# PinataFarms/FEARTracker

Hardware: AMD Instinct MI355X
Metric: search-region crops/sec (FEAR-XS 256x256) (higher is better)
Workload: dtype f32; 1 GPU; FEAR-XS track(): batch=256 synthetic 256x256 search / 128x128 template crops per GPU, fp32; batch_per_gpu=256, global_batch=256, weights=FEAR-XS-NoEmbs (fp16 values upcast to fp32), engine_pass=256, parallelism=dp1, math=fp32 MFMA (v_mfma_f32_16x16x4_f32), exact fp32

## Files before the change

### feartracker_amd/csrc/fear_e1pair.h

```cpp
#pragma once
#include <type_traits>
#include <vector>

#ifndef E1P_NA
#define E1P_NA 3
#endif

namespace fear {

struct E1PairArgs {
    const float* X;
    float* Y;
    const float* Wpk;
    int H, W, tiles_x, tiles_y;
    int tpw;
};

struct E1PairGeom {
    static constexpr int C = 24, T = 16, XW = T + 4, MW = T + 2, NQ = C / 4;
    static constexpr int XPL = XW * XW * 4;
    static constexpr int XSKEW = 12;
    static constexpr int xb(int q) { return q * XPL + (q >> 1) * XSKEW; }
    static constexpr int XT_FLOATS = NQ * XPL + 2 * XSKEW;
    static constexpr int NSLOT = NQ * XW * XW, NIT = (NSLOT + 511) / 512;
    static constexpr int MPL = (MW * MW * 4 + 63) / 64 * 64;
    static constexpr int NPIX_A = MW * MW, NMT_A = (NPIX_A + 15) / 16, MTA = (NMT_A + 7) / 8;
    static constexpr int FRAG = 4 * 256, TAP0 = FRAG, TAP1 = TAP0 + 9 * 16, BD = TAP1 + 9 * 8, BP = BD + 24, WBLK = BP + 32;
    static constexpr int WS = WBLK - FRAG;
    static_assert(WS % 4 == 0 && WBLK % 4 == 0, "16-byte granules");
    static constexpr int LDS_FLOATS = XT_FLOATS + NQ * MPL + 2 * WS;
    static constexpr int LDS_BYTES = LDS_FLOATS * 4;
};

inline void e1pair_pack_block(std::vector<float>& out, const float* dw, const float* bd, const float* pw, const float* bp) {
    using G = E1PairGeom;
    for (int c = 0; c < 2; ++c)
        for (int nt = 0; nt < 2; ++nt)
            for (int l = 0; l < 64; ++l)
                for (int i = 0; i < 4; ++i) {
                    const int n = nt * 16 + (l & 15);
                    const int k = c == 0 ? (l >> 4) * 4 + i : (i < 2 ? 16 + 2 * (l >> 4) + i : G::C);
                    out.push_back(n < G::C && k < G::C ? pw[n * G::C + k] : 0.f);
                }
    for (int t = 0; t < 9; ++t)
        for (int ch = 0; ch < 16; ++ch) out.push_back(dw[ch * 9 + t]);
    for (int t = 0; t < 9; ++t)
        for (int ch = 16; ch < 24; ++ch) out.push_back(dw[ch * 9 + t]);
    for (int ch = 0; ch < 24; ++ch) out.push_back(bd ? bd[ch] : 0.f);
    for (int ch = 0; ch < 32; ++ch) out.push_back(ch < 24 ? bp[ch] : 0.f);
}

__device__ __forceinline__ void pk_fma2(f32x2& d, const f32x2& a, const f32x2& b) {
    asm volatile("v_pk_fma_f32 %0, %1, %2, %0" : "+v"(d) : "v"(a), "v"(b));
}

__device__ __forceinline__ void e1_project(f32x4 d4, f32x2 d2, const f32x4 (&wp)[4], const f32x4 (&bias)[2], f32x4 (&acc)[2]) {
    d4.x = fmaxf(d4.x, 0.f); d4.y = fmaxf(d4.y, 0.f); d4.z = fmaxf(d4.z, 0.f); d4.w = fmaxf(d4.w, 0.f);
    d2.x = fmaxf(d2.x, 0.f); d2.y = fmaxf(d2.y, 0.f);
#pragma unroll
    for (int nt = 0; nt < 2; ++nt) {
        f32x4 a = bias[nt];
#pragma unroll
        for (int q = 0; q < 4; ++q) a = __builtin_amdgcn_mfma_f32_16x16x4f32(wp[nt][q], d4[q], a, 0, 0, 0);
#pragma unroll
        for (int q = 0; q < 2; ++q) a = __builtin_amdgcn_mfma_f32_16x16x4f32(wp[2 + nt][q], d2[q], a, 0, 0, 0);
        acc[nt] = a;
    }
}

__device__ __forceinline__ int e1_fill_slot(int tid) {
    const int l = tid & 63, g = l >> 3, j = l & 7;
    return (tid & ~63) | (8 * ((g + j) & 7) + j);
}

template <int IT0, int IT1>
__device__ __forceinline__ void e1_issue_loads(const E1PairArgs& a, unsigned tix, int tid, f32x4 (&xv)[E1PairGeom::NIT]) {
    using G = E1PairGeom;
    constexpr int T = G::T, XW = G::XW, NQ = G::NQ, C = G::C;
    const int tiles = a.tiles_x * a.tiles_y;
    const long crop = tix / tiles;
    const int tile = tix % tiles;
    const int ox0 = (tile % a.tiles_x) * T, oy0 = (tile / a.tiles_x) * T;
    const float* Xc = a.X + crop * a.H * a.W * C;
    const __amdgpu_buffer_rsrc_t img = __builtin_amdgcn_make_buffer_rsrc(const_cast<float*>(Xc), 0, a.H * a.W * C * 4, 0x00020000);
    int t = e1_fill_slot(tid);
    asm volatile("" : "+v"(t));
#pragma unroll
    for (int it = IT0; it < IT1; ++it) {
        const int s = it * 512 + t;
        const int pix = s / NQ, q = s - pix * NQ;
        const int py = pix / XW, px = pix - py * XW;
        const int gy = oy0 - 2 + py, gx = ox0 - 2 + px;
        const bool ok = s < G::NSLOT && gy >= 0 && gy < a.H && gx >= 0 && gx < a.W;
        xv[it] = __builtin_bit_cast(f32x4, __builtin_amdgcn_raw_buffer_load_b128(img, ok ? ((gy * a.W + gx) * C + q * 4) * 4 : (int)0x80000000, 0, 0));
    }
}
template <int IT0, int IT1>
__device__ __forceinline__ void e1_commit_tile(float* Xt, int tid, const f32x4 (&xv)[E1PairGeom::NIT]) {
    using G = E1PairGeom;
    int t = e1_fill_slot(tid);
    asm volatile("" : "+v"(t));
#pragma unroll
    for (int it = IT0; it < IT1; ++it) {
        const int s = it * 512 + t;
        const int pix = s / G::NQ, q = s - pix * G::NQ;
        if (s < G::NSLOT) *reinterpret_cast<f32x4*>(Xt + q * G::XPL + (q >> 1) * G::XSKEW + pix * 4) = xv[it];
    }
}

__global__ __launch_bounds__(512, 4) void e1pair_kernel(E1PairArgs a) {
    using G = E1PairGeom;
    constexpr int T = G::T, XW = G::XW, MW = G::MW, XPL = G::XPL, MPL = G::MPL, NQ = G::NQ, C = G::C;
    extern __shared__ __attribute__((aligned(16))) float lds[];
    float* const Xt = lds;
    float* const Mt = lds + G::XT_FLOATS;
    float* const WSl = Mt + NQ * MPL;
    const int tid = threadIdx.x, lane = tid & 63;
    const int wave = __builtin_amdgcn_readfirstlane(tid >> 6);
    const int li = lane & 15, lk = lane >> 4;
    const int tiles = a.tiles_x * a.tiles_y;
    const int tpw = a.tpw > 0 ? a.tpw : 1;
    const unsigned t_first = xcd_tile_index(blockIdx.x, gridDim.x) * (unsigned)tpw;

    constexpr int NIT = G::NIT;
    constexpr int NA = E1P_NA;
    f32x4 xv0[NIT];
    e1_issue_loads<0, NIT>(a, t_first, tid, xv0);
    auto load_wp = [&](int b, f32x4 (&wp)[4]) {
#pragma unroll
        for (int f = 0; f < 4; ++f) wp[f] = *reinterpret_cast<const f32x4*>(a.Wpk + b * G::WBLK + f * 256 + lane * 4);
    };
    if (tid < 2 * G::WS / 4) {
        const int b = tid / (G::WS / 4), j = tid - b * (G::WS / 4);
        *reinterpret_cast<f32x4*>(WSl + b * G::WS + j * 4) = *reinterpret_cast<const f32x4*>(a.Wpk + b * G::WBLK + G::FRAG + j * 4);
    }
    e1_commit_tile<0, NIT>(Xt, tid, xv0);

    for (int ti = 0; ti < tpw; ++ti) {
        const unsigned tix = t_first + ti;
        const long crop = tix / tiles;
        const int tile = tix % tiles;
        const int ox0 = (tile % a.tiles_x) * T, oy0 = (tile / a.tiles_x) * T;
        float* Yc = a.Y + crop * a.H * a.W * C;
        __syncthreads();
        f32x4 xv[NIT];
        int li_o = li, lk_o = lk;
        asm volatile("" : "+v"(li_o), "+v"(lk_o));
        if (ti + 1 < tpw) e1_issue_loads<0, NA>(a, tix + 1, tid, xv);

        {
            const float* ws = WSl;
            f32x4 wp[4];
            load_wp(0, wp);
            auto block_a = [&](auto nm_tag) {
                constexpr int NM = decltype(nm_tag)::value;
                int pc[NM], cpix[NM];
                bool valid[NM];
                float inside[NM];
#pragma unroll
                for (int i = 0; i < NM; ++i) {
                    const int mt = wave + 8 * i;
                    const int j = (mt - MW) * 16 + li_o;
                    valid[i] = mt < MW || j < 2 * MW;
                    const int my = mt < MW ? mt : (valid[i] ? j >> 1 : 0), mx = mt < MW ? li_o : 16 + (j & 1);
                    pc[i] = my * MW + mx;
                    cpix[i] = (my + 1) * XW + mx + 1;
                    const int gy = oy0 - 1 + my, gx = ox0 - 1 + mx;
                    inside[i] = (gy >= 0 && gy < a.H && gx >= 0 && gx < a.W) ? 1.f : 0.f;
                }
                f32x4 d4[NM];
                f32x2 d2[NM];
                {
                    const f32x4 b0 = *reinterpret_cast<const f32x4*>(ws + (G::BD - G::FRAG) + lk_o * 4);
                    const f32x2 b1 = *reinterpret_cast<const f32x2*>(ws + (G::BD - G::FRAG) + 16 + lk_o * 2);
#pragma unroll
                    for (int i = 0; i < NM; ++i) { d4[i] = b0; d2[i] = b1; }
                }
                const float* s0 = Xt + lk_o * XPL + (lk_o >> 1) * G::XSKEW;
                const float* s1 = Xt + (4 + (lk_o >> 1)) * XPL + 2 * G::XSKEW + (lk_o & 1) * 2;
#pragma unroll
                for (int k = 0; k < 9; ++k) {
                    const f32x4 w4 = *reinterpret_cast<const f32x4*>(ws + (G::TAP0 - G::FRAG) + k * 16 + lk_o * 4);
                    const f32x2 w2 = *reinterpret_cast<const f32x2*>(ws + (G::TAP1 - G::FRAG) + k * 8 + lk_o * 2);
                    const int off = ((k / 3 - 1) * XW + (k % 3 - 1)) * 4;
#pragma unroll
                    for (int i = 0; i < NM; ++i) {
                        const f32x4 v4 = *reinterpret_cast<const f32x4*>(s0 + cpix[i] * 4 + off);
                        const f32x2 v2 = *reinterpret_cast<const f32x2*>(s1 + cpix[i] * 4 + off);
                        pk_fma4(d4[i], v4, w4);
                        pk_fma2(d2[i], v2, w2);
                    }
                }
                f32x4 bpv[2];
#pragma unroll
                for (int nt = 0; nt < 2; ++nt) bpv[nt] = *reinterpret_cast<const f32x4*>(ws + (G::BP - G::FRAG) + (nt * 4 + lk_o) * 4);
#pragma unroll
                for (int i = 0; i < NM; ++i) {
                    f32x4 acc[2];
                    e1_project(d4[i], d2[i], wp, bpv, acc);
#pragma unroll
                    for (int nt = 0; nt < 2; ++nt) {
                        if (nt == 1 && lk_o >= 2) continue;
                        const int qd = nt * 4 + lk_o;
                        const f32x4 v = (acc[nt] + *reinterpret_cast<const f32x4*>(Xt + qd * XPL + (qd >> 1) * G::XSKEW + cpix[i] * 4)) * inside[i];
                        if (valid[i]) *reinterpret_cast<f32x4*>(Mt + qd * MPL + pc[i] * 4) = v;
                    }
                }
            };
            if (wave + 16 < G::NMT_A) block_a(std::integral_constant<int, 3>{});
            else block_a(std::integral_constant<int, 2>{});
        }
        __syncthreads();
        if (ti + 1 < tpw) { e1_commit_tile<0, NA>(Xt, tid, xv); e1_issue_loads<NA, NIT>(a, tix + 1, tid, xv); }

        {
            const float* ws = WSl + G::WS;
            f32x4 wp[4];
            load_wp(1, wp);
            f32x4 bpv[2];
#pragma unroll
            for (int nt = 0; nt < 2; ++nt) bpv[nt] = *reinterpret_cast<const f32x4*>(ws + (G::BP - G::FRAG) + (nt * 4 + lk_o) * 4);
            const int row0 = wave * 2;
            const int cpix = (row0 + 1) * MW + li_o + 1;
            f32x4 d4[2];
            f32x2 d2[2];
            d4[0] = d4[1] = *reinterpret_cast<const f32x4*>(ws + (G::BD - G::FRAG) + lk_o * 4);
            d2[0] = d2[1] = *reinterpret_cast<const f32x2*>(ws + (G::BD - G::FRAG) + 16 + lk_o * 2);
            {
                const float* s0 = Mt + lk_o * MPL + cpix * 4;
                const float* s1 = Mt + (4 + (lk_o >> 1)) * MPL + cpix * 4 + (lk_o & 1) * 2;
                f32x4 w4[2][3];
                f32x2 w2[2][3];
#pragma unroll
                for (int iy = 0; iy < 4; ++iy) {
#pragma unroll
                    for (int kx = 0; kx < 3; ++kx) {
                        if (iy < 3) {
                            w4[iy & 1][kx] = *reinterpret_cast<const f32x4*>(ws + (G::TAP0 - G::FRAG) + (iy * 3 + kx) * 16 + lk_o * 4);
                            w2[iy & 1][kx] = *reinterpret_cast<const f32x2*>(ws + (G::TAP1 - G::FRAG) + (iy * 3 + kx) * 8 + lk_o * 2);
                        }
                        const int off = ((iy - 1) * MW + (kx - 1)) * 4;
                        const f32x4 v4 = *reinterpret_cast<const f32x4*>(s0 + off);
                        const f32x2 v2 = *reinterpret_cast<const f32x2*>(s1 + off);
                        if (iy < 3) { pk_fma4(d4[0], v4, w4[iy & 1][kx]); pk_fma2(d2[0], v2, w2[iy & 1][kx]); }
                        if (iy >= 1) { pk_fma4(d4[1], v4, w4[(iy - 1) & 1][kx]); pk_fma2(d2[1], v2, w2[(iy - 1) & 1][kx]); }
                    }
                }
            }
            const unsigned ylane = (unsigned)(li_o * C + lk_o * 4);
#pragma unroll
            for (int r = 0; r < 2; ++r) {
                f32x4 acc[2];
                e1_project(d4[r], d2[r], wp, bpv, acc);
                float* yrow = Yc + ((long)(oy0 + row0 + r) * a.W + ox0) * C;
#pragma unroll
                for (int nt = 0; nt < 2; ++nt) {
                    if (nt == 1 && lk_o >= 2) continue;
                    const int qd = nt * 4 + lk_o;
                    const f32x4 v = acc[nt] + *reinterpret_cast<const f32x4*>(Mt + qd * MPL + (cpix + r * MW) * 4);
                    *reinterpret_cast<f32x4*>(yrow + (ylane + (unsigned)(nt * 16))) = v;
                }
            }
        }
        if (ti + 1 < tpw) e1_commit_tile<NA, NIT>(Xt, tid, xv);
    }
}

}
```

### feartracker_amd/csrc/fear_engine.hip

```cpp
#include <hip/hip_runtime.h>

#include <atomic>
#include <cstdio>
#include <cstdlib>
#include <cstring>
#include <map>
#include <memory>
#include <mutex>
#include <string>
#include <vector>

#include "../../include/fear_hip.h"
#include "../../include/fearw_format.h"
#include "fear_kernels.h"
#include "fear_headchain.h"
#include "fear_headchain_b.h"
#include "fear_e1pair.h"
#include "fear_chain32.h"
#include "fear_yuv.h"
#ifndef FEAR_E1PAIR_TPW_MAX
#define FEAR_E1PAIR_TPW_MAX 1
#endif

namespace {

using namespace fear;

float half_to_float(uint16_t h) {
    const uint32_t sign = (uint32_t)(h & 0x8000u) << 16;
    uint32_t exp = (h >> 10) & 0x1f;
    uint32_t man = h & 0x3ffu;
    uint32_t bits;
    if (exp == 0) {
        if (man == 0) {
            bits = sign;
        } else {
            int e = -1;
            do { ++e; man <<= 1; } while (!(man & 0x400u));
            bits = sign | ((uint32_t)(127 - 15 - e) << 23) | ((man & 0x3ffu) << 13);
        }
    } else if (exp == 31) {
        bits = sign | 0x7f800000u | (man << 13);
    } else {
        bits = sign | ((exp + 127 - 15) << 23) | (man << 13);
    }
    float f;
    memcpy(&f, &bits, 4);
    return f;
}

uint16_t float_to_half(float f) {
    uint32_t x;
    memcpy(&x, &f, 4);
    const uint32_t sign = (x >> 16) & 0x8000u;
    const int32_t e = (int32_t)((x >> 23) & 0xff) - 127 + 15;
    uint32_t man = x & 0x7fffffu;
    if (((x >> 23) & 0xff) == 0xff) return (uint16_t)(sign | 0x7c00u | (man ? 0x200u : 0));
    if (e >= 31) return (uint16_t)(sign | 0x7c00u);
    if (e <= 0) {
        if (e < -10) return (uint16_t)sign;
        man |= 0x800000u;
        const int shift = 14 - e;
        uint32_t h = man >> shift;
        const uint32_t rem = man & ((1u << shift) - 1), half = 1u << (shift - 1);
        if (rem > half || (rem == half && (h & 1))) ++h;
        return (uint16_t)(sign | h);
    }
    uint32_t h = ((uint32_t)e << 10) | (man >> 13);
    const uint32_t rem = man & 0x1fffu;
    if (rem > 0x1000u || (rem == 0x1000u && (h & 1))) ++h;
    return (uint16_t)(sign | h);
}

uint16_t float_to_bf16(float f) {
    uint32_t x;
    memcpy(&x, &f, 4);
    if ((x & 0x7f800000u) == 0x7f800000u) return (uint16_t)((x >> 16) | ((x & 0xffffu) ? 0x40u : 0));
    x += 0x7fffu + ((x >> 16) & 1u);
    return (uint16_t)(x >> 16);
}

struct Conv {
    int cout, cin_g, groups, k, stride, pad, relu, has_bias;
    std::vector<float> w;
    std::vector<float> b;
    float* d_w = nullptr;
    float* d_w2 = nullptr;
    float* d_b = nullptr;
    bool is_dw() const { return groups == cout && cin_g == 1 && groups > 1; }
    bool is_pw() const { return groups == 1 && k == 1; }
};

struct Fused16Row;
struct TileRow;
struct TileK;

enum OpType { OP_STEM, OP_PW, OP_DW, OP_CORR, OP_PW_SMALL, OP_IR16, OP_IRTILE, OP_CHAIN16, OP_HEADCHAIN, OP_E1PAIR, OP_CHAIN32, OP_CHAIN32_16 };

struct Op {
    OpType type;
    int conv = -1;
    int in_buf = -1, in_ld = 0, in_off = 0;
    int out_buf = -1, out_ld = 0, out_off = 0;
    int res_buf = -1, res_ld = 0;
    int H = 0, W = 0;
    int Ho = 0, Wo = 0;
    int C = 0, N = 0;
    int relu = 0, act = 0;
    int out_external = 0;
    int tmpl_cls = 0;
    int pred_fused = 0;
    float* pred_packed = nullptr;
    int pred_conv_p = -1;
    int pw_split = 0;
    int splitk = 0;
    int tiny = 0;
    int nsplit = 0;
    int part_buf = -1;
    int lane = 0;
    int corr_fused = 0;
    int conv_e = -1, conv_d = -1, conv_p = -1;
    int relu_dw = 0;
    const Fused16Row* f16 = nullptr;
    const TileRow* tile = nullptr;
    const TileK* tk = nullptr;
    float* d_packed = nullptr;
    int math = 0;
    int pred_cout = 0;
    int stem = 0;
    int io_bf16 = 0;
    float* chain_pk[8] = {nullptr};
    int chain_cp[8] = {0};
    float* chain16_pk[8] = {nullptr};
    int chain16_cp[8] = {0};
    float* neck_pk = nullptr;
    int neck_conv = -1;
    float* hc_w[2][4] = {{nullptr}};
    float* hc_wd0[2] = {nullptr};
    float* hc_wdc[2] = {nullptr};
    float* hc_pred[2] = {nullptr};
    float* hc_taps[2][4] = {{nullptr}};
    int hc_pred_conv[2] = {-1, -1};
    int hc_pred_act[2] = {0, 0};
    char name[64];
    double flops = 0, bytes = 0;
    std::vector<std::pair<hipEvent_t, hipEvent_t>> events;
    double prof_ms = 0;
    int64_t prof_n = 0;
};

enum class PlanKind {
    Throughput,
    Small,
    Tiny,
    MidSize,
};

struct Plan {
    bool with_head = false;
    bool small = false;
    std::vector<Op> ops;
    int head_first = -1;
    int n_bufs = 0;
    size_t buf_floats_per_crop = 0;
};

}

struct fear_handle {
    int device = 0;
    std::vector<Conv> convs;
    std::vector<FearwBlock> blocks;
    bool has_head = false;
    int feat_channels = 0;
    int max_batch = 64;
// ... 1222 lines not shown
                if (!h->event_pool.empty()) { *e = h->event_pool.back(); h->event_pool.pop_back(); }
                else HIP_TRY(h, hipEventCreate(e));
            }
            HIP_TRY(h, hipEventRecord(e0, s));
        }
        const Conv* c = op.conv >= 0 ? &h->convs[op.conv] : nullptr;
        switch (op.type) {
            case OP_STEM: {
                if (h->fuse && op.Wo % 16 == 0) {
                    StemMfmaArgs a{ext.img, c->d_w2, c->d_b, buf(op.out_buf), n, op.H, op.W, op.Ho, op.Wo};
                    const long rows = (long)n * op.Ho;
                    hipLaunchKernelGGL(stem_mfma_kernel, dim3((rows + 3) / 4), dim3(256), 0, s, a);
                } else {
                    StemArgs a{ext.img, c->d_w, c->d_b, buf(op.out_buf), n, op.H, op.W, op.Ho, op.Wo};
                    const long total = (long)n * op.Ho * op.Wo;
                    hipLaunchKernelGGL(stem_conv_kernel, dim3((total + 255) / 256), dim3(256), 0, s, a);
                }
                break;
            }
            case OP_PW: {
                PwArgs a{};
                a.X = buf(op.in_buf) + op.in_off; a.ldx = op.in_ld;
                a.W = c->d_w; a.bias = c->d_b;
                a.R = op.res_buf >= 0 ? buf(op.res_buf) : nullptr; a.ldr = op.res_ld;
                a.M = n * op.H * op.W; a.K = op.C; a.N = op.N; a.relu = op.relu;
                if (op.out_external == 1) { a.Y = ext.feat_out; a.ldy = op.N; a.nchw_hw = op.H * op.W; }
                else { a.Y = buf(op.out_buf) + op.out_off; a.ldy = op.out_ld; a.nchw_hw = 0; }
                const int n_tiles = (op.N + 15) / 16;
                int nt = pick_nt(n_tiles);
                const int rows_per_block = 4 * 2 * 16;
                dim3 grid((a.M + rows_per_block - 1) / rows_per_block);
                if (op.pw_split && n_tiles % 2 == 0) {
                    grid.y = n_tiles / 2;
                    hipLaunchKernelGGL((pw_mfma_kernel<2, 2, false, 8>), grid, dim3(256), 0, s, a);
                    break;
                }
                if (h->math && p.with_head) launch_pw_h<false>(h->math, n_tiles, grid, s, a);
                else launch_pw_nt<2, false>(nt, grid, s, a);
                break;
            }
            case OP_CORR: {
                PwArgs a{};
                a.X = buf(op.in_buf) + op.in_off; a.ldx = op.in_ld;
                a.W = (op.tmpl_cls && ext.tmpl_cls) ? ext.tmpl_cls : ext.tmpl;
                a.bias = nullptr; a.R = nullptr;
                a.Y = buf(op.out_buf) + op.out_off; a.ldy = op.out_ld;
                a.M = n * op.H * op.W; a.K = op.C; a.N = op.N; a.relu = 0; a.nchw_hw = 0;
                a.rows_per_crop = op.H * op.W; a.w_crop_stride = (long)op.C * op.N;
                const int rows_per_block = 4 * 2 * 16;
                dim3 grid((a.M + rows_per_block - 1) / rows_per_block);
                int nt = pick_nt(op.N / 16);
                if (op.pw_split) {
                    grid.x = (a.M + 63) / 64;
                    grid.y = op.N / 16;
                    if (a.K <= 256) hipLaunchKernelGGL((pw_mfma_kernel<1, 1, true, 16>), grid, dim3(256), 0, s, a);
                    else hipLaunchKernelGGL((pw_mfma_kernel<1, 1, true, 8>), grid, dim3(256), 0, s, a);
                    break;
                }
                if (h->math) launch_pw_h<true>(h->math, op.N / 16, grid, s, a);
                else launch_pw_nt<2, true>(nt, grid, s, a);
                break;
            }
            case OP_DW: {
                DwArgs a{};
                a.X = buf(op.in_buf) + op.in_off; a.ldx = op.in_ld;
                a.Wt = c->d_w; a.bias = c->d_b;
                a.Y = buf(op.out_buf); a.ldy = op.out_ld;
                a.B = n; a.H = op.H; a.W = op.W; a.C = op.C; a.Ho = op.Ho; a.Wo = op.Wo; a.relu = op.relu;
                const long strips = (op.Ho + 3) / 4;
                const long total = (long)n * strips * op.Wo * (op.C / 4);
                dim3 grid((total + 255) / 256);
                launch_dw(c->k, c->stride, grid, s, a);
                break;
            }
            case OP_IR16: {
                const Fused16Row& r = *op.f16;
                const F16K& f = r.by_math(op.math);
                Ir2Args a{};
                a.X = buf(op.in_buf) + op.in_off; a.ldx = op.in_ld;
                a.Wpk = op.d_packed; a.bp = h->convs[op.conv_p].d_b;
                a.R = op.res_buf >= 0 ? buf(op.res_buf) : nullptr; a.ldr = op.res_ld;
                a.Y = op.out_buf >= 0 ? buf(op.out_buf) : nullptr; a.ldy = op.out_ld;
                a.relu_dw = op.relu_dw; a.relu_out = op.relu;
                if (op.pred_cout > 0) {
                    a.pred_cout = op.pred_cout; a.pred_act = op.act;
                    a.pred_stride = op.out_external == 3 ? ext.cls_stride : ext.bbox_stride;
                    float* y = op.out_external == 3 ? ext.cls_out : ext.bbox_out;
                    if (op.pred_fused) { a.P_Wpk = op.pred_packed; a.P_bp = h->convs[op.pred_conv_p].d_b; a.P_Y = y; }
                    else a.Y = y;
                }
                if (op.nsplit) {
                    const Conv& dconv = h->convs[op.conv_d];
                    a.nsplit_wstride = (long)(dconv.cout / 16) * (256 + dconv.k * dconv.k * 16 + 16);
                    if (op.tiny) hipLaunchKernelGGL(r.tiny.kernel, dim3(n, op.nsplit, 16 / kTinyRows), dim3(64 * kTinyRows * kTinyKSplit), r.tiny.lds_bytes, s, a);
                    else hipLaunchKernelGGL(f.kernel, dim3(n, op.nsplit), dim3(512), f.lds_bytes, s, a);
                } else if (op.tiny) {
                    hipLaunchKernelGGL(r.tiny.kernel, dim3(n, 1, 16 / kTinyRows), dim3(64 * kTinyRows * kTinyKSplit), r.tiny.lds_bytes, s, a);
                } else if (op.splitk) {
                    Ir2Args pa = a;
                    const Conv& dconv = h->convs[op.conv_d];
                    pa.kc_count = dconv.cout / 16 / op.splitk;
                    pa.Y = buf(op.part_buf); pa.ldy = op.N;
                    pa.kc_part_stride = (long)n * 256 * op.N;
                    pa.R = nullptr;
                    hipLaunchKernelGGL(r.splitk.kernel, dim3(n, op.splitk), dim3(512), r.splitk.lds_bytes, s, pa);
                    SplitKReduceArgs ra{};
                    ra.P = pa.Y; ra.bias = a.bp; ra.R = a.R; ra.Y = a.Y; ra.part_stride = pa.kc_part_stride;
                    ra.W = op.splitk; ra.M = n * 256; ra.N = op.N; ra.ldp = op.N; ra.ldr = a.ldr; ra.ldy = a.ldy; ra.relu = a.relu_out;
                    const long total = (long)ra.M * (ra.N / 4);
                    hipLaunchKernelGGL(splitk_reduce_kernel, dim3((unsigned)((total + 255) / 256)), dim3(256), 0, s, ra);
                } else if (op.corr_fused) {
                    a.Z = (op.tmpl_cls && ext.tmpl_cls) ? ext.tmpl_cls : ext.tmpl;
                    a.z_stride = (long)kCorrC * kCorrTz;
                    hipLaunchKernelGGL(kSep16CorrKernel, dim3(n), dim3(512), kSep16CorrLds, s, a);
                } else if (op.pred_fused) {
                    hipLaunchKernelGGL(kSep16PredKernel, dim3(n), dim3(512), kSep16PredLds, s, a);
                } else {
                    hipLaunchKernelGGL(f.kernel, dim3(n), dim3(512), f.lds_bytes, s, a);
                }
                break;
            }
            case OP_IRTILE: {
                const TileK& f = *op.tk;
                IrT2Args ta{};
                Ir2Args& a = ta.b;
                if (op.stem) { a.X = ext.img; a.ldx = 0; }
                else { a.X = buf(op.in_buf) + op.in_off; a.ldx = op.in_ld; }
                a.Wpk = op.d_packed; a.bp = h->convs[op.conv_p].d_b;
                a.R = op.res_buf >= 0 ? buf(op.res_buf) : nullptr; a.ldr = op.res_ld;
                a.Y = buf(op.out_buf); a.ldy = op.out_ld;
                a.relu_dw = op.relu_dw; a.relu_out = op.relu;
                ta.H = op.H; ta.W = op.W; ta.tiles_x = op.Wo / f.tw; ta.tiles_y = op.Ho / f.th;
                if (op.splitk) {
                    const TileK& ks = op.tile->ksplit;
                    SplitKReduceArgs ra{};
                    ra.bias = a.bp; ra.R = a.R; ra.Y = a.Y; ra.W = op.splitk; ra.M = n * op.Ho * op.Wo; ra.N = op.N; ra.ldp = op.N;
                    ra.ldr = a.ldr; ra.ldy = a.ldy; ra.relu = a.relu_out;
                    ra.part_stride = (long)ra.M * op.N;
                    a.Y = buf(op.part_buf); a.ldy = op.N; a.R = nullptr; a.kc_part_stride = ra.part_stride;
                    ra.P = a.Y;
                    hipLaunchKernelGGL(ks.kernel, dim3((unsigned)n * ta.tiles_x * ta.tiles_y, op.splitk), dim3(512), ks.lds_bytes, s, ta);
                    const long total = (long)ra.M * (ra.N / 4);
                    hipLaunchKernelGGL(splitk_reduce_kernel, dim3((unsigned)((total + 255) / 256)), dim3(256), 0, s, ra);
                    break;
                }
                const TileK& k = op.io_bf16 ? *op.tile->io_variant(op.io_bf16) : f;
                hipLaunchKernelGGL(k.kernel, dim3((unsigned)n * ta.tiles_x * ta.tiles_y), dim3(64 * k.nw), k.lds_bytes, s, ta);
                break;
            }
            case OP_E1PAIR: {
                E1PairArgs a{};
                a.X = buf(op.in_buf); a.Y = buf(op.out_buf); a.Wpk = op.d_packed;
                a.H = op.H; a.W = op.W; a.tiles_x = op.W / E1PairGeom::T; a.tiles_y = op.H / E1PairGeom::T;
                const unsigned total = (unsigned)n * a.tiles_x * a.tiles_y;
                a.tpw = 1;
                for (int t = FEAR_E1PAIR_TPW_MAX; t > 1; t >>= 1)
                    if (total % t == 0 && total / t >= 512) { a.tpw = t; break; }
                hipLaunchKernelGGL(e1pair_kernel, dim3(total / a.tpw), dim3(512), E1PairGeom::LDS_BYTES, s, a);
                break;
            }
            case OP_CHAIN16: {
                Chain16Args a{};
                a.X = buf(op.in_buf) + op.in_off; a.ldx = op.in_ld;
                a.Y = buf(op.out_buf); a.ldy = op.out_ld;
                for (int j = 0; j < 7; ++j) { a.Wpk[j] = op.chain_pk[j]; a.bp[j] = h->convs[op.chain_cp[j]].d_b; }
                a.neck_pk = op.neck_pk; a.neck_b = h->convs[op.neck_conv].d_b;
                hipLaunchKernelGGL(kChainXSKernel, dim3(n), dim3(512), kChainXSLds, s, a);
                break;
            }
            case OP_CHAIN32: {
                Chain32Args a{};
                a.X = buf(op.in_buf) + op.in_off; a.ldx = op.in_ld;
                a.Y = buf(op.out_buf); a.ldy = op.out_ld;
                for (int j = 0; j < 4; ++j) { a.Wpk[j] = op.chain_pk[j]; a.bp[j] = h->convs[op.chain_cp[j]].d_b; }
                hipLaunchKernelGGL(kChain32XSKernel, dim3(n), dim3(512), C32Geom::LDS_BYTES, s, a);
                break;
            }
            case OP_CHAIN32_16: {
                Chain32Args a{};
                a.X = buf(op.in_buf) + op.in_off; a.ldx = op.in_ld;
                a.Y = nullptr; a.ldy = 0;
                for (int j = 0; j < 4; ++j) { a.Wpk[j] = op.chain_pk[j]; a.bp[j] = h->convs[op.chain_cp[j]].d_b; }
                Chain16Args b{};
                b.X = nullptr; b.ldx = 0;
                b.Y = buf(op.out_buf); b.ldy = op.out_ld;
                for (int j = 0; j < 7; ++j) { b.Wpk[j] = op.chain16_pk[j]; b.bp[j] = h->convs[op.chain16_cp[j]].d_b; }
                b.neck_pk = op.neck_pk; b.neck_b = h->convs[op.neck_conv].d_b;
                hipLaunchKernelGGL(kChain32_16XSKernel, dim3(n), dim3(512), kChain32_16Lds, s, a, b);
                break;
            }
            case OP_HEADCHAIN: {
                if (op.math == 2) {
                    HeadChainBArgs a{};
                    a.X = buf(op.in_buf) + op.in_off; a.ldx = op.in_ld; a.n_crops = n;
                    a.relu_dw = op.relu_dw; a.relu_out = op.relu;
                    for (int br = 0; br < 2; ++br) {
                        HeadChainBBranch& b = a.br[br];
                        for (int l = 0; l < 4; ++l) { b.W[l] = op.hc_w[br][l]; b.Wd[l] = op.hc_taps[br][l]; }
                        b.Z = (br == 0 && ext.tmpl_cls) ? ext.tmpl_cls : ext.tmpl;
                        b.z_stride = (long)HeadChainG::C * HeadChainG::TZ;
                        b.P_W = op.hc_pred[br]; b.P_bp = h->convs[op.hc_pred_conv[br]].d_b;
                        b.P_Y = br == 0 ? ext.cls_out : ext.bbox_out;
                        b.pred_stride = br == 0 ? ext.cls_stride : ext.bbox_stride;
                        b.pred_cout = br == 0 ? 1 : 4; b.pred_act = op.hc_pred_act[br];
                    }
                    hipLaunchKernelGGL(kHeadChainBKernel, dim3(16u * ((unsigned)(n + 7) / 8)), dim3(512), HeadChainBG::LDS_BYTES, s, a);
                    break;
                }
                HeadChainArgs a{};
                a.X = buf(op.in_buf) + op.in_off; a.ldx = op.in_ld; a.n_crops = n;
                a.relu_dw = op.relu_dw; a.relu_out = op.relu;
                for (int br = 0; br < 2; ++br) {
                    HeadChainBranch& b = a.br[br];
                    for (int l = 0; l < 4; ++l) b.W[l] = op.hc_w[br][l];
                    b.Wd0 = op.hc_wd0[br]; b.WdC = op.hc_wdc[br];
                    b.Z = (br == 0 && ext.tmpl_cls) ? ext.tmpl_cls : ext.tmpl;
                    b.z_stride = (long)HeadChainG::C * HeadChainG::TZ;
                    b.P_Wpk = op.hc_pred[br]; b.P_bp = h->convs[op.hc_pred_conv[br]].d_b;
                    b.P_Y = br == 0 ? ext.cls_out : ext.bbox_out;
                    b.pred_stride = br == 0 ? ext.cls_stride : ext.bbox_stride;
                    b.pred_cout = br == 0 ? 1 : 4; b.pred_act = op.hc_pred_act[br];
                    b.D = buf(op.out_buf) + (size_t)br * n * HeadChainG::D_FLOATS;
                }
                hipLaunchKernelGGL(kHeadChainKernel, dim3(16u * ((unsigned)(n + 7) / 8)), dim3(512), HeadChainG::LDS_BYTES, s, a);
                break;
            }
            case OP_PW_SMALL: {
                PwSmallArgs a{};
                a.X = buf(op.in_buf); a.ldx = op.in_ld; a.W = c->d_w; a.bias = c->d_b;
                a.Y = op.out_external == 3 ? ext.cls_out : ext.bbox_out;
                a.M = n * op.H * op.W; a.K = op.C; a.N = op.N; a.hw = op.H * op.W; a.act = op.act;
                a.crop_stride = op.out_external == 3 ? ext.cls_stride : ext.bbox_stride;
                dim3 grid(((long)a.M * 16 + 255) / 256);
                if (op.N == 1) hipLaunchKernelGGL((pw_small_kernel<1>), grid, dim3(256), 0, s, a);
                else hipLaunchKernelGGL((pw_small_kernel<4>), grid, dim3(256), 0, s, a);
                break;
            }
        }
        if (prof) {
            HIP_TRY(h, hipEventRecord(e1, s));
            op.events.emplace_back(e0, e1);
        }
    }
    if (forked) {
        HIP_TRY(h, hipEventRecord(h->branch_join, h->branch_stream));
        HIP_TRY(h, hipStreamWaitEvent(s_main, h->branch_join, 0));
    }
    HIP_TRY(h, hipGetLastError());
    return FEAR_OK;
}

int drain_events(fear_handle* h) {
    for (auto& kv : h->plans)
        for (Op& op : kv.second->ops) {
            for (auto& ev : op.events) {
                HIP_TRY(h, hipEventSynchronize(ev.second));
                float ms = 0.f;
                HIP_TRY(h, hipEventElapsedTime(&ms, ev.first, ev.second));
                op.prof_ms += ms;
                op.prof_n += 1;
                h->event_pool.push_back(ev.first);
                h->event_pool.push_back(ev.second);
            }
            op.events.clear();
        }
    return FEAR_OK;
}

int drop_plans(fear_handle* h) {
    if (h->plans.empty() && h->plan_allocs.empty()) return FEAR_OK;
    HIP_TRY(h, hipSetDevice(h->device));
    HIP_TRY(h, hipDeviceSynchronize());
    const int st = drain_events(h);
    if (st != FEAR_OK) return st;
    h->plans.clear();
    for (float* p : h->plan_allocs) hipFree(p);
    h->plan_allocs.clear();
    return FEAR_OK;
}

struct OptionDesc {
    int option;
    int fear_handle::*field;
    int64_t min, max;
    bool rebuilds_plans;
};
const OptionDesc kOptions[] = {
    {FEAR_OPT_MAX_BATCH, &fear_handle::max_batch, 1, 65536, false},
    {FEAR_OPT_PROFILE, &fear_handle::profile, 0, 1, false},
    {FEAR_OPT_PROFILE_OP, &fear_handle::profile_op, -1, 4096, false},
    {FEAR_OPT_FUSE, &fear_handle::fuse, 0, 1, true},
    {FEAR_OPT_MATH, &fear_handle::math, 0, 2, true},
    {FEAR_OPT_CHAIN, &fear_handle::chain, 0, 1, true},
    {FEAR_OPT_SMALL_PASS, &fear_handle::small_pass, 0, 65536, false},
    {FEAR_OPT_PLAN_CROPS, &fear_handle::plan_crops, 0, 65536, false},
    {FEAR_OPT_DUAL_HEAD, &fear_handle::dual_head, 0, 1, true},
    {FEAR_OPT_TILE_V4, &fear_handle::tile_v4, 0, 1, true},
    {FEAR_OPT_TINY_SEP, &fear_handle::tiny_sep, 0, 1, true},
    {FEAR_OPT_HEAD_STAGGER, &fear_handle::head_stagger_us, 0, 1000, false},
    {FEAR_OPT_HEAD_CHAIN, &fear_handle::head_chain, 0, 1, true},
    {FEAR_OPT_E1_PAIR, &fear_handle::e1_pair, 0, 1, true},
    {FEAR_OPT_CHAIN32, &fear_handle::chain32, 0, 2, true},
    {FEAR_OPT_BF16_STORE, &fear_handle::bf16_store, 0, 1, true},
    {FEAR_OPT_SPLIT_STREAMS, &fear_handle::split_streams, 0, 1, false},
};
const OptionDesc* find_option(int option) {
    for (const OptionDesc& d : kOptions)
        if (d.option == option) return &d;
    return nullptr;
}

// ... 401 lines not shown
```

Baseline: 118,400 crops/s.

## Simplify e1pair to one tile per block with row-based buffer fills

Drops the multi-tile-per-block software pipeline, which was inactive by default since TPW_MAX was 1, so each block now handles a single tile. The halo fill is reorganised so two waves load one input row, using per-row buffer resources with a scalar row offset and a lane-skewed slot order, replacing per-slot divides and bounds checks. Stage A precomputes LDS pointers per output row and splits row and column sub-tiles, and the per-lane weight offsets are hoisted into registers. The aim is less address arithmetic and fewer VGPRs in the fill and stencil loops, and the fill now depends on RSLOT fitting within 128 slots.

Measured after the change: 118,900 crops/s (median of 6 runs). Within noise of the previous version (+0.4%).

```diff
diff --git a/feartracker_amd/csrc/fear_e1pair.h b/feartracker_amd/csrc/fear_e1pair.h
--- a/feartracker_amd/csrc/fear_e1pair.h
+++ b/feartracker_amd/csrc/fear_e1pair.h
@@ -2,8 +2,10 @@
 #include <type_traits>
 #include <vector>
 
-#ifndef E1P_NA
-#define E1P_NA 3
+#if defined(__HIPCC__)
+#define E1P_HD __host__ __device__
+#else
+#define E1P_HD
 #endif
 
 namespace fear {
@@ -13,16 +15,17 @@
     float* Y;
     const float* Wpk;
     int H, W, tiles_x, tiles_y;
-    int tpw;
 };
 
 struct E1PairGeom {
     static constexpr int C = 24, T = 16, XW = T + 4, MW = T + 2, NQ = C / 4;
     static constexpr int XPL = XW * XW * 4;
     static constexpr int XSKEW = 12;
-    static constexpr int xb(int q) { return q * XPL + (q >> 1) * XSKEW; }
+    static constexpr E1P_HD int xb(int q) { return q * XPL + (q >> 1) * XSKEW; }
     static constexpr int XT_FLOATS = NQ * XPL + 2 * XSKEW;
-    static constexpr int NSLOT = NQ * XW * XW, NIT = (NSLOT + 511) / 512;
+    static constexpr int RSLOT = NQ * XW;
+    static constexpr int NSLOT = RSLOT * XW, NIT = XW / 4;
+    static_assert(XW % 4 == 0 && RSLOT <= 128, "eight waves fill four rows per pass, two waves a row");
     static constexpr int MPL = (MW * MW * 4 + 63) / 64 * 64;
     static constexpr int NPIX_A = MW * MW, NMT_A = (NPIX_A + 15) / 16, MTA = (NMT_A + 7) / 8;
     static constexpr int FRAG = 4 * 256, TAP0 = FRAG, TAP1 = TAP0 + 9 * 16, BD = TAP1 + 9 * 8, BP = BD + 24, WBLK = BP + 32;
@@ -31,6 +34,36 @@
     static constexpr int LDS_FLOATS = XT_FLOATS + NQ * MPL + 2 * WS;
     static constexpr int LDS_BYTES = LDS_FLOATS * 4;
 };
+
+constexpr E1P_HD int e1_fill_slot_of_lane(int lane) { return (lane * 9) & 63; }
+constexpr E1P_HD int e1_fill_row_slot(int tid) { return ((tid >> 6) & 1) * 64 + e1_fill_slot_of_lane(tid & 63); }
+constexpr E1P_HD int e1_fill_pix(int tid) { return e1_fill_row_slot(tid) / E1PairGeom::NQ; }
+constexpr E1P_HD int e1_fill_quad(int tid) { return e1_fill_row_slot(tid) % E1PairGeom::NQ; }
+constexpr E1P_HD int e1_fill_row(int tid, int it) { return it * 4 + (tid >> 7); }
+constexpr E1P_HD int e1_fill_lds_thread(int tid) {
+    return E1PairGeom::xb(e1_fill_quad(tid)) + ((tid >> 7) * E1PairGeom::XW + e1_fill_pix(tid)) * 4;
+}
+constexpr E1P_HD int e1_fill_lds_pass(int it) { return it * 4 * E1PairGeom::XW * 4; }
+constexpr E1P_HD int e1_fill_base_bytes(int ox0) { return (ox0 - 2) * E1PairGeom::C * 4; }
+constexpr E1P_HD int e1_fill_row_bytes(int gy, int W) { return gy * W * E1PairGeom::C * 4; }
+constexpr E1P_HD int e1_fill_lane_bytes(int tid) { return e1_fill_row_slot(tid) * 16; }
+constexpr E1P_HD bool e1_fill_lane_ok(int tid, int ox0, int W) {
+    const int gx = ox0 - 2 + e1_fill_pix(tid);
+    return e1_fill_row_slot(tid) < E1PairGeom::RSLOT && gx >= 0 && gx < W;
+}
+constexpr E1P_HD bool e1_fill_row_ok(int tid, int it, int oy0, int H) {
+    const int gy = oy0 - 2 + e1_fill_row(tid, it);
+    return gy >= 0 && gy < H;
+}
+
+constexpr E1P_HD int e1_a_row_xpix(int wave, int li) { return (wave + 1) * E1PairGeom::XW + li + 1; }
+constexpr E1P_HD int e1_a_row_mpix(int wave, int li) { return wave * E1PairGeom::MW + li; }
+struct E1ColLane { bool valid; int my, mx; };
+constexpr E1P_HD E1ColLane e1_a_col_lane(int c, int li) {
+    const int j = c * 16 + li;
+    const bool valid = j < 2 * E1PairGeom::MW;
+    return {valid, valid ? j >> 1 : 0, 16 + (j & 1)};
+}
 
 inline void e1pair_pack_block(std::vector<float>& out, const float* dw, const float* bd, const float* pw, const float* bp) {
     using G = E1PairGeom;
@@ -50,6 +83,8 @@
     for (int ch = 0; ch < 32; ++ch) out.push_back(ch < 24 ? bp[ch] : 0.f);
 }
 
+#if defined(__HIPCC__)
+
 __device__ __forceinline__ void pk_fma2(f32x2& d, const f32x2& a, const f32x2& b) {
     asm volatile("v_pk_fma_f32 %0, %1, %2, %0" : "+v"(d) : "v"(a), "v"(b));
 }
@@ -68,49 +103,9 @@
     }
 }
 
-__device__ __forceinline__ int e1_fill_slot(int tid) {
-    const int l = tid & 63, g = l >> 3, j = l & 7;
-    return (tid & ~63) | (8 * ((g + j) & 7) + j);
-}
-
-template <int IT0, int IT1>
-__device__ __forceinline__ void e1_issue_loads(const E1PairArgs& a, unsigned tix, int tid, f32x4 (&xv)[E1PairGeom::NIT]) {
-    using G = E1PairGeom;
-    constexpr int T = G::T, XW = G::XW, NQ = G::NQ, C = G::C;
-    const int tiles = a.tiles_x * a.tiles_y;
-    const long crop = tix / tiles;
-    const int tile = tix % tiles;
-    const int ox0 = (tile % a.tiles_x) * T, oy0 = (tile / a.tiles_x) * T;
-    const float* Xc = a.X + crop * a.H * a.W * C;
-    const __amdgpu_buffer_rsrc_t img = __builtin_amdgcn_make_buffer_rsrc(const_cast<float*>(Xc), 0, a.H * a.W * C * 4, 0x00020000);
-    int t = e1_fill_slot(tid);
-    asm volatile("" : "+v"(t));
-#pragma unroll
-    for (int it = IT0; it < IT1; ++it) {
-        const int s = it * 512 + t;
-        const int pix = s / NQ, q = s - pix * NQ;
-        const int py = pix / XW, px = pix - py * XW;
-        const int gy = oy0 - 2 + py, gx = ox0 - 2 + px;
-        const bool ok = s < G::NSLOT && gy >= 0 && gy < a.H && gx >= 0 && gx < a.W;
-        xv[it] = __builtin_bit_cast(f32x4, __builtin_amdgcn_raw_buffer_load_b128(img, ok ? ((gy * a.W + gx) * C + q * 4) * 4 : (int)0x80000000, 0, 0));
-    }
-}
-template <int IT0, int IT1>
-__device__ __forceinline__ void e1_commit_tile(float* Xt, int tid, const f32x4 (&xv)[E1PairGeom::NIT]) {
-    using G = E1PairGeom;
-    int t = e1_fill_slot(tid);
-    asm volatile("" : "+v"(t));
-#pragma unroll
-    for (int it = IT0; it < IT1; ++it) {
-        const int s = it * 512 + t;
-        const int pix = s / G::NQ, q = s - pix * G::NQ;
-        if (s < G::NSLOT) *reinterpret_cast<f32x4*>(Xt + q * G::XPL + (q >> 1) * G::XSKEW + pix * 4) = xv[it];
-    }
-}
-
 __global__ __launch_bounds__(512, 4) void e1pair_kernel(E1PairArgs a) {
     using G = E1PairGeom;
-    constexpr int T = G::T, XW = G::XW, MW = G::MW, XPL = G::XPL, MPL = G::MPL, NQ = G::NQ, C = G::C;
+    constexpr int T = G::T, XW = G::XW, MW = G::MW, XPL = G::XPL, MPL = G::MPL, NQ = G::NQ, C = G::C, NIT = G::NIT;
     extern __shared__ __attribute__((aligned(16))) float lds[];
     float* const Xt = lds;
     float* const Mt = lds + G::XT_FLOATS;
@@ -119,151 +114,181 @@
     const int wave = __builtin_amdgcn_readfirstlane(tid >> 6);
     const int li = lane & 15, lk = lane >> 4;
     const int tiles = a.tiles_x * a.tiles_y;
-    const int tpw = a.tpw > 0 ? a.tpw : 1;
-    const unsigned t_first = xcd_tile_index(blockIdx.x, gridDim.x) * (unsigned)tpw;
-
-    constexpr int NIT = G::NIT;
-    constexpr int NA = E1P_NA;
-    f32x4 xv0[NIT];
-    e1_issue_loads<0, NIT>(a, t_first, tid, xv0);
+    const unsigned tix = xcd_tile_index(blockIdx.x, gridDim.x);
+    const long crop = tix / tiles;
+    const int tile = tix % tiles;
+    const int ox0 = (tile % a.tiles_x) * T, oy0 = (tile / a.tiles_x) * T;
+    const float* Xc = a.X + crop * a.H * a.W * C;
+    float* Yc = a.Y + crop * a.H * a.W * C;
+
+    {
+        const int ftid = wave * 64 + lane;
+        const int voff = e1_fill_lane_ok(ftid, ox0, a.W) ? e1_fill_lane_bytes(ftid) : (int)0x80000000;
+        const char* xrow0 = reinterpret_cast<const char*>(Xc) + e1_fill_base_bytes(ox0);
+        f32x4 xv[NIT];
+#pragma unroll
+        for (int it = 0; it < NIT; ++it) {
+            const bool rok = e1_fill_row_ok(wave * 64, it, oy0, a.H);
+            const int gy = oy0 - 2 + e1_fill_row(wave * 64, it);
+            const int soff = rok ? e1_fill_row_bytes(gy, a.W) : 0;
+            const __amdgpu_buffer_rsrc_t img = __builtin_amdgcn_make_buffer_rsrc(const_cast<char*>(xrow0), 0, rok ? soff + G::RSLOT * 16 : 0, 0x00020000);
+            xv[it] = __builtin_bit_cast(f32x4, __builtin_amdgcn_raw_buffer_load_b128(img, voff, soff, 0));
+        }
+        if (tid < 2 * G::WS / 4) {
+            const int b = tid >= G::WS / 4 ? 1 : 0, j = tid - b * (G::WS / 4);
+            *reinterpret_cast<f32x4*>(WSl + b * G::WS + j * 4) = *reinterpret_cast<const f32x4*>(a.Wpk + b * G::WBLK + G::FRAG + j * 4);
+        }
+        if (e1_fill_row_slot(ftid) < G::RSLOT) {
+            float* xdst = Xt + e1_fill_lds_thread(ftid);
+#pragma unroll
+            for (int it = 0; it < NIT; ++it) *reinterpret_cast<f32x4*>(xdst + e1_fill_lds_pass(it)) = xv[it];
+        }
+    }
     auto load_wp = [&](int b, f32x4 (&wp)[4]) {
 #pragma unroll
         for (int f = 0; f < 4; ++f) wp[f] = *reinterpret_cast<const f32x4*>(a.Wpk + b * G::WBLK + f * 256 + lane * 4);
     };
-    if (tid < 2 * G::WS / 4) {
-        const int b = tid / (G::WS / 4), j = tid - b * (G::WS / 4);
-        *reinterpret_cast<f32x4*>(WSl + b * G::WS + j * 4) = *reinterpret_cast<const f32x4*>(a.Wpk + b * G::WBLK + G::FRAG + j * 4);
-    }
-    e1_commit_tile<0, NIT>(Xt, tid, xv0);
-
-    for (int ti = 0; ti < tpw; ++ti) {
-        const unsigned tix = t_first + ti;
-        const long crop = tix / tiles;
-        const int tile = tix % tiles;
-        const int ox0 = (tile % a.tiles_x) * T, oy0 = (tile / a.tiles_x) * T;
-        float* Yc = a.Y + crop * a.H * a.W * C;
-        __syncthreads();
-        f32x4 xv[NIT];
-        int li_o = li, lk_o = lk;
-        asm volatile("" : "+v"(li_o), "+v"(lk_o));
-        if (ti + 1 < tpw) e1_issue_loads<0, NA>(a, tix + 1, tid, xv);
-
+    int wq = G::XT_FLOATS + NQ * MPL + lk * 4, wh = G::XT_FLOATS + NQ * MPL + lk * 2;
+    asm volatile("" : "+v"(wq), "+v"(wh));
+    __syncthreads();
+
+    {
+        const float* ws4 = lds + wq;
+        const float* ws2 = lds + wh;
+        f32x4 wp[4];
+        load_wp(0, wp);
+        auto block_a = [&](auto nr_tag, auto nc_tag) {
+            constexpr int NR = decltype(nr_tag)::value, NC = decltype(nc_tag)::value, NM = NR + NC;
+            const int xcorner = (e1_a_row_xpix(wave, li) - XW - 1) * 4;
+            const float* s0[NM];
+            const float* s1[NM];
+            const float* r1[NM];
+            float* m0[NM];
+            float inside[NM];
+            bool valid = true;
+            {
+                const float* p0 = Xt + G::xb(lk);
+                const float* p1 = Xt + G::xb(4 + (lk >> 1)) + (lk & 1) * 2;
+                const float* pr = Xt + G::xb(4 + lk);
+                float* pm = Mt + lk * MPL;
+                const int gxr = ox0 - 1 + li;
+                const float colf = (gxr >= 0 && gxr < a.W) ? 1.f : 0.f;
+#pragma unroll
+                for (int i = 0; i < NR; ++i) {
+                    s0[i] = p0 + xcorner + i * 8 * XW * 4;
+                    s1[i] = p1 + xcorner + i * 8 * XW * 4;
+                    r1[i] = pr + xcorner + i * 8 * XW * 4;
+                    m0[i] = pm + e1_a_row_mpix(wave, li) * 4 + i * 8 * MW * 4;
+                    const int gy = oy0 - 1 + wave + 8 * i;
+                    inside[i] = (gy >= 0 && gy < a.H) ? colf : 0.f;
+                }
+                if constexpr (NC > 0) {
+                    const E1ColLane cl = e1_a_col_lane(wave + 8 * NR - MW, li);
+                    valid = cl.valid;
+                    const int ccorner = (cl.my * XW + cl.mx) * 4;
+                    s0[NR] = p0 + ccorner;
+                    s1[NR] = p1 + ccorner;
+                    r1[NR] = pr + ccorner;
+                    m0[NR] = pm + (cl.my * MW + cl.mx) * 4;
+                    const int gy = oy0 - 1 + cl.my, gx = ox0 - 1 + cl.mx;
+                    inside[NR] = (gy >= 0 && gy < a.H && gx >= 0 && gx < a.W) ? 1.f : 0.f;
+                }
+            }
+            f32x4 d4[NM];
+            f32x2 d2[NM];
+            {
+                const f32x4 b0 = *reinterpret_cast<const f32x4*>(ws4 + (G::BD - G::FRAG));
+                const f32x2 b1 = *reinterpret_cast<const f32x2*>(ws2 + (G::BD - G::FRAG) + 16);
+#pragma unroll
+                for (int i = 0; i < NM; ++i) { d4[i] = b0; d2[i] = b1; }
+            }
+#pragma unroll
+            for (int k = 0; k < 9; ++k) {
+                const f32x4 w4 = *reinterpret_cast<const f32x4*>(ws4 + (G::TAP0 - G::FRAG) + k * 16);
+                const f32x2 w2 = *reinterpret_cast<const f32x2*>(ws2 + (G::TAP1 - G::FRAG) + k * 8);
+                const int off = ((k / 3) * XW + (k % 3)) * 4;
+#pragma unroll
+                for (int i = 0; i < NM; ++i) {
+                    const f32x4 v4 = *reinterpret_cast<const f32x4*>(s0[i] + off);
+                    const f32x2 v2 = *reinterpret_cast<const f32x2*>(s1[i] + off);
+                    pk_fma4(d4[i], v4, w4);
+                    pk_fma2(d2[i], v2, w2);
+                }
+            }
+            f32x4 bpv[2];
+#pragma unroll
+            for (int nt = 0; nt < 2; ++nt) bpv[nt] = *reinterpret_cast<const f32x4*>(ws4 + (G::BP - G::FRAG) + nt * 16);
+            constexpr int ctr = (XW + 1) * 4;
+#pragma unroll
+            for (int i = 0; i < NM; ++i) {
+                f32x4 acc[2];
+                e1_project(d4[i], d2[i], wp, bpv, acc);
+#pragma unroll
+                for (int nt = 0; nt < 2; ++nt) {
+                    if (nt == 1 && lk >= 2) continue;
+                    const f32x4 v = (acc[nt] + *reinterpret_cast<const f32x4*>((nt ? r1[i] : s0[i]) + ctr)) * inside[i];
+                    if (i < NR || valid) *reinterpret_cast<f32x4*>(m0[i] + nt * 4 * MPL) = v;
+                }
+            }
+        };
+        using std::integral_constant;
+        if (wave + 16 < MW) block_a(integral_constant<int, 3>{}, integral_constant<int, 0>{});
+        else if (wave + 16 < G::NMT_A) block_a(integral_constant<int, 2>{}, integral_constant<int, 1>{});
+        else block_a(integral_constant<int, 2>{}, integral_constant<int, 0>{});
+    }
+    __syncthreads();
+
+    {
+        const float* ws4 = lds + wq + G::WS;
+        const float* ws2 = lds + wh + G::WS;
+        f32x4 wp[4];
+        load_wp(1, wp);
+        f32x4 bpv[2];
+#pragma unroll
+        for (int nt = 0; nt < 2; ++nt) bpv[nt] = *reinterpret_cast<const f32x4*>(ws4 + (G::BP - G::FRAG) + nt * 16);
+        const int row0 = wave * 2;
+        const int corner = (row0 * MW + li) * 4;
+        f32x4 d4[2];
+        f32x2 d2[2];
+        d4[0] = d4[1] = *reinterpret_cast<const f32x4*>(ws4 + (G::BD - G::FRAG));
+        d2[0] = d2[1] = *reinterpret_cast<const f32x2*>(ws2 + (G::BD - G::FRAG) + 16);
+        const float* s0 = Mt + lk * MPL + corner;
         {
-            const float* ws = WSl;
-            f32x4 wp[4];
-            load_wp(0, wp);
-            auto block_a = [&](auto nm_tag) {
-                constexpr int NM = decltype(nm_tag)::value;
-                int pc[NM], cpix[NM];
-                bool valid[NM];
-                float inside[NM];
-#pragma unroll
-                for (int i = 0; i < NM; ++i) {
-                    const int mt = wave + 8 * i;
-                    const int j = (mt - MW) * 16 + li_o;
-                    valid[i] = mt < MW || j < 2 * MW;
-                    const int my = mt < MW ? mt : (valid[i] ? j >> 1 : 0), mx = mt < MW ? li_o : 16 + (j & 1);
-                    pc[i] = my * MW + mx;
-                    cpix[i] = (my + 1) * XW + mx + 1;
-                    const int gy = oy0 - 1 + my, gx = ox0 - 1 + mx;
-                    inside[i] = (gy >= 0 && gy < a.H && gx >= 0 && gx < a.W) ? 1.f : 0.f;
-                }
-                f32x4 d4[NM];
-                f32x2 d2[NM];
-                {
-                    const f32x4 b0 = *reinterpret_cast<const f32x4*>(ws + (G::BD - G::FRAG) + lk_o * 4);
-                    const f32x2 b1 = *reinterpret_cast<const f32x2*>(ws + (G::BD - G::FRAG) + 16 + lk_o * 2);
-#pragma unroll
-                    for (int i = 0; i < NM; ++i) { d4[i] = b0; d2[i] = b1; }
-                }
-                const float* s0 = Xt + lk_o * XPL + (lk_o >> 1) * G::XSKEW;
-                const float* s1 = Xt + (4 + (lk_o >> 1)) * XPL + 2 * G::XSKEW + (lk_o & 1) * 2;
-#pragma unroll
-                for (int k = 0; k < 9; ++k) {
-                    const f32x4 w4 = *reinterpret_cast<const f32x4*>(ws + (G::TAP0 - G::FRAG) + k * 16 + lk_o * 4);
-                    const f32x2 w2 = *reinterpret_cast<const f32x2*>(ws + (G::TAP1 - G::FRAG) + k * 8 + lk_o * 2);
-                    const int off = ((k / 3 - 1) * XW + (k % 3 - 1)) * 4;
-#pragma unroll
-                    for (int i = 0; i < NM; ++i) {
-                        const f32x4 v4 = *reinterpret_cast<const f32x4*>(s0 + cpix[i] * 4 + off);
-                        const f32x2 v2 = *reinterpret_cast<const f32x2*>(s1 + cpix[i] * 4 + off);
-                        pk_fma4(d4[i], v4, w4);
-                        pk_fma2(d2[i], v2, w2);
+            const float* s1 = Mt + (4 + (lk >> 1)) * MPL + corner + (lk & 1) * 2;
+            f32x4 w4[2][3];
+            f32x2 w2[2][3];
+#pragma unroll
+            for (int iy = 0; iy < 4; ++iy) {
+#pragma unroll
+                for (int kx = 0; kx < 3; ++kx) {
+                    if (iy < 3) {
+                        w4[iy & 1][kx] = *reinterpret_cast<const f32x4*>(ws4 + (G::TAP0 - G::FRAG) + (iy * 3 + kx) * 16);
+                        w2[iy & 1][kx] = *reinterpret_cast<const f32x2*>(ws2 + (G::TAP1 - G::FRAG) + (iy * 3 + kx) * 8);
                     }
-                }
-                f32x4 bpv[2];
-#pragma unroll
-                for (int nt = 0; nt < 2; ++nt) bpv[nt] = *reinterpret_cast<const f32x4*>(ws + (G::BP - G::FRAG) + (nt * 4 + lk_o) * 4);
-#pragma unroll
-                for (int i = 0; i < NM; ++i) {
-                    f32x4 acc[2];
-                    e1_project(d4[i], d2[i], wp, bpv, acc);
-#pragma unroll
-                    for (int nt = 0; nt < 2; ++nt) {
-                        if (nt == 1 && lk_o >= 2) continue;
-                        const int qd = nt * 4 + lk_o;
-                        const f32x4 v = (acc[nt] + *reinterpret_cast<const f32x4*>(Xt + qd * XPL + (qd >> 1) * G::XSKEW + cpix[i] * 4)) * inside[i];
-                        if (valid[i]) *reinterpret_cast<f32x4*>(Mt + qd * MPL + pc[i] * 4) = v;
-                    }
-                }
-            };
-            if (wave + 16 < G::NMT_A) block_a(std::integral_constant<int, 3>{});
-            else block_a(std::integral_constant<int, 2>{});
-        }
-        __syncthreads();
-        if (ti + 1 < tpw) { e1_commit_tile<0, NA>(Xt, tid, xv); e1_issue_loads<NA, NIT>(a, tix + 1, tid, xv); }
-
-        {
-            const float* ws = WSl + G::WS;
-            f32x4 wp[4];
-            load_wp(1, wp);
-            f32x4 bpv[2];
-#pragma unroll
-            for (int nt = 0; nt < 2; ++nt) bpv[nt] = *reinterpret_cast<const f32x4*>(ws + (G::BP - G::FRAG) + (nt * 4 + lk_o) * 4);
-            const int row0 = wave * 2;
-            const int cpix = (row0 + 1) * MW + li_o + 1;
-            f32x4 d4[2];
-            f32x2 d2[2];
-            d4[0] = d4[1] = *reinterpret_cast<const f32x4*>(ws + (G::BD - G::FRAG) + lk_o * 4);
-            d2[0] = d2[1] = *reinterpret_cast<const f32x2*>(ws + (G::BD - G::FRAG) + 16 + lk_o * 2);
-            {
-                const float* s0 = Mt + lk_o * MPL + cpix * 4;
-                const float* s1 = Mt + (4 + (lk_o >> 1)) * MPL + cpix * 4 + (lk_o & 1) * 2;
-                f32x4 w4[2][3];
-                f32x2 w2[2][3];
-#pragma unroll
-                for (int iy = 0; iy < 4; ++iy) {
-#pragma unroll
-                    for (int kx = 0; kx < 3; ++kx) {
-                        if (iy < 3) {
-                            w4[iy & 1][kx] = *reinterpret_cast<const f32x4*>(ws + (G::TAP0 - G::FRAG) + (iy * 3 + kx) * 16 + lk_o * 4);
-                            w2[iy & 1][kx] = *reinterpret_cast<const f32x2*>(ws + (G::TAP1 - G::FRAG) + (iy * 3 + kx) * 8 + lk_o * 2);
-                        }
-                        const int off = ((iy - 1) * MW + (kx - 1)) * 4;
-                        const f32x4 v4 = *reinterpret_cast<const f32x4*>(s0 + off);
-                        const f32x2 v2 = *reinterpret_cast<const f32x2*>(s1 + off);
-                        if (iy < 3) { pk_fma4(d4[0], v4, w4[iy & 1][kx]); pk_fma2(d2[0], v2, w2[iy & 1][kx]); }
-                        if (iy >= 1) { pk_fma4(d4[1], v4, w4[(iy - 1) & 1][kx]); pk_fma2(d2[1], v2, w2[(iy - 1) & 1][kx]); }
-                    }
-                }
-            }
-            const unsigned ylane = (unsigned)(li_o * C + lk_o * 4);
-#pragma unroll
-            for (int r = 0; r < 2; ++r) {
-                f32x4 acc[2];
-                e1_project(d4[r], d2[r], wp, bpv, acc);
-                float* yrow = Yc + ((long)(oy0 + row0 + r) * a.W + ox0) * C;
-#pragma unroll
-                for (int nt = 0; nt < 2; ++nt) {
-                    if (nt == 1 && lk_o >= 2) continue;
-                    const int qd = nt * 4 + lk_o;
-                    const f32x4 v = acc[nt] + *reinterpret_cast<const f32x4*>(Mt + qd * MPL + (cpix + r * MW) * 4);
-                    *reinterpret_cast<f32x4*>(yrow + (ylane + (unsigned)(nt * 16))) = v;
-                }
-            }
-        }
-        if (ti + 1 < tpw) e1_commit_tile<NA, NIT>(Xt, tid, xv);
-    }
-}
-
-}
+                    const int off = (iy * MW + kx) * 4;
+                    const f32x4 v4 = *reinterpret_cast<const f32x4*>(s0 + off);
+                    const f32x2 v2 = *reinterpret_cast<const f32x2*>(s1 + off);
+                    if (iy < 3) { pk_fma4(d4[0], v4, w4[iy & 1][kx]); pk_fma2(d2[0], v2, w2[iy & 1][kx]); }
+                    if (iy >= 1) { pk_fma4(d4[1], v4, w4[(iy - 1) & 1][kx]); pk_fma2(d2[1], v2, w2[(iy - 1) & 1][kx]); }
+                }
+            }
+        }
+        const unsigned ylane = (unsigned)(li * C + lk * 4);
+#pragma unroll
+        for (int r = 0; r < 2; ++r) {
+            f32x4 acc[2];
+            e1_project(d4[r], d2[r], wp, bpv, acc);
+            float* yrow = Yc + ((long)(oy0 + row0 + r) * a.W + ox0) * C;
+#pragma unroll
+            for (int nt = 0; nt < 2; ++nt) {
+                if (nt == 1 && lk >= 2) continue;
+                const f32x4 v = acc[nt] + *reinterpret_cast<const f32x4*>(s0 + nt * 4 * MPL + ((r + 1) * MW + 1) * 4);
+                *reinterpret_cast<f32x4*>(yrow + (ylane + (unsigned)(nt * 16))) = v;
+            }
+        }
+    }
+}
+
+#endif
+
+}
diff --git a/feartracker_amd/csrc/fear_engine.hip b/feartracker_amd/csrc/fear_engine.hip
--- a/feartracker_amd/csrc/fear_engine.hip
+++ b/feartracker_amd/csrc/fear_engine.hip
@@ -18,9 +18,6 @@
 #include "fear_e1pair.h"
 #include "fear_chain32.h"
 #include "fear_yuv.h"
-#ifndef FEAR_E1PAIR_TPW_MAX
-#define FEAR_E1PAIR_TPW_MAX 1
-#endif
 
 namespace {
 
@@ -1549,11 +1546,7 @@
                 E1PairArgs a{};
                 a.X = buf(op.in_buf); a.Y = buf(op.out_buf); a.Wpk = op.d_packed;
                 a.H = op.H; a.W = op.W; a.tiles_x = op.W / E1PairGeom::T; a.tiles_y = op.H / E1PairGeom::T;
-                const unsigned total = (unsigned)n * a.tiles_x * a.tiles_y;
-                a.tpw = 1;
-                for (int t = FEAR_E1PAIR_TPW_MAX; t > 1; t >>= 1)
-                    if (total % t == 0 && total / t >= 512) { a.tpw = t; break; }
-                hipLaunchKernelGGL(e1pair_kernel, dim3(total / a.tpw), dim3(512), E1PairGeom::LDS_BYTES, s, a);
+                hipLaunchKernelGGL(e1pair_kernel, dim3((unsigned)n * a.tiles_x * a.tiles_y), dim3(512), E1PairGeom::LDS_BYTES, s, a);
                 break;
             }
             case OP_CHAIN16: {
```
